# OwshenNetwork/owshen

Hardware: NVIDIA H100
Metric: groth16_withdraw_proofs_per_sec (higher is better)
Workload: dtype u256 (8x32-bit Montgomery limbs, integer)

## Files before the change

### owshen_b200/csrc/ec.cuh

```cuda
#pragma once
#include "fp.cuh"

namespace og {

template <class F>
struct Affine {
    F x, y;
    OG_HD static Affine inf() { return Affine{F::zero(), F::zero()}; }
    OG_HD bool is_inf() const { return x.is_zero() && y.is_zero(); }
    OG_HD Affine neg() const { return Affine{x, y.neg()}; }
    OG_HD bool operator==(const Affine& o) const { return x == o.x && y == o.y; }
};

template <class F>
struct XYZZ {
    F x, y, zz, zzz;

    OG_HD static XYZZ inf() { return XYZZ{F::one(), F::one(), F::zero(), F::zero()}; }
    OG_HD bool is_inf() const { return zz.is_zero(); }
    OG_HD static XYZZ from_affine(const Affine<F>& p) {
        if (p.is_inf()) return inf();
        return XYZZ{p.x, p.y, F::one(), F::one()};
    }
    OG_HD XYZZ neg() const { return XYZZ{x, y.neg(), zz, zzz}; }

    OG_HD static XYZZ dbl_affine(const Affine<F>& p) {
        F u = p.y.dbl();
        F v = u.sqr();
        F w = u * v;
        F s = p.x * v;
        F xx = p.x.sqr();
        F m = xx.dbl() + xx;
        F x3 = m.sqr() - s.dbl();
        F y3 = m * (s - x3) - w * p.y;
        return XYZZ{x3, y3, v, w};
    }

    OG_HD XYZZ dbl() const {
        if (is_inf()) return *this;
        F u = y.dbl();
        F v = u.sqr();
        F w = u * v;
        F s = x * v;
        F xx = x.sqr();
        F m = xx.dbl() + xx;
        F x3 = m.sqr() - s.dbl();
        F y3 = m * (s - x3) - w * y;
        return XYZZ{x3, y3, v * zz, w * zzz};
    }

    OG_HD void madd(const Affine<F>& q) {
        if (q.is_inf()) return;
        if (is_inf()) { x = q.x; y = q.y; zz = F::one(); zzz = F::one(); return; }
        F u2 = q.x * zz;
        F s2 = q.y * zzz;
        F p = u2 - x;
        F r = s2 - y;
        if (p.is_zero()) {
            if (r.is_zero()) *this = dbl_affine(q);
            else *this = inf();
            return;
        }
        F pp = p.sqr();
        F ppp = p * pp;
        F q1 = x * pp;
        F x3 = r.sqr() - ppp - q1.dbl();
        y = r * (q1 - x3) - y * ppp;
        x = x3;
        zz = zz * pp;
        zzz = zzz * ppp;
    }

    OG_HD void add(const XYZZ& o) {
        if (o.is_inf()) return;
        if (is_inf()) { *this = o; return; }
        F u1 = x * o.zz;
        F u2 = o.x * zz;
        F s1 = y * o.zzz;
        F s2 = o.y * zzz;
        F p = u2 - u1;
        F r = s2 - s1;
        if (p.is_zero()) {
            if (r.is_zero()) *this = dbl();
            else *this = inf();
            return;
        }
        F pp = p.sqr();
        F ppp = p * pp;
        F q1 = u1 * pp;
        F x3 = r.sqr() - ppp - q1.dbl();
        y = r * (q1 - x3) - s1 * ppp;
        x = x3;
        zz = zz * o.zz * pp;
        zzz = zzz * o.zzz * ppp;
    }

    OG_HD Affine<F> to_affine() const {
        if (is_inf()) return Affine<F>::inf();
        F t = (zz * zzz).inv();
        return Affine<F>{x * (t * zzz), y * (t * zz)};
    }

    OG_HD static XYZZ mul(const Affine<F>& p, const uint32_t* k) {
        XYZZ acc = inf();
        for (int i = 255; i >= 0; i--) {
            acc = acc.dbl();
            if ((k[i >> 5] >> (i & 31)) & 1) acc.madd(p);
        }
        return acc;
    }
};

#if defined(__CUDACC__)
template <class F> __device__ __noinline__ void xyzz_add_ni(XYZZ<F>* a, const XYZZ<F>* b) { a->add(*b); }
template <class F> __device__ __noinline__ void xyzz_madd_ni(XYZZ<F>* a, const Affine<F>* b) { a->madd(*b); }
template <class F> __device__ __noinline__ void xyzz_dbl_ni(XYZZ<F>* a) { *a = a->dbl(); }
template <class F> __device__ __noinline__ void xyzz_to_affine_ni(Affine<F>* r, const XYZZ<F>* a) { *r = a->to_affine(); }
#endif

typedef Affine<Fq> G1Affine;
typedef Affine<Fq2> G2Affine;
typedef XYZZ<Fq> G1XYZZ;
typedef XYZZ<Fq2> G2XYZZ;

}
```

### owshen_b200/csrc/fp.cuh

```cuda
#pragma once
#include <stdint.h>
#include <string.h>

#if defined(__CUDACC__)
#define OG_HD __host__ __device__ __forceinline__
#else
#define OG_HD inline
#endif

namespace og {

struct CC { uint32_t c = 0; };

#if defined(__CUDA_ARCH__)
#define OG_ASM asm volatile
OG_HD uint32_t add_cc(uint32_t a, uint32_t b, CC&) { uint32_t r; OG_ASM("add.cc.u32 %0, %1, %2;" : "=r"(r) : "r"(a), "r"(b)); return r; }
OG_HD uint32_t addc_cc(uint32_t a, uint32_t b, CC&) { uint32_t r; OG_ASM("addc.cc.u32 %0, %1, %2;" : "=r"(r) : "r"(a), "r"(b)); return r; }
OG_HD uint32_t addc(uint32_t a, uint32_t b, CC&) { uint32_t r; OG_ASM("addc.u32 %0, %1, %2;" : "=r"(r) : "r"(a), "r"(b)); return r; }
OG_HD uint32_t sub_cc(uint32_t a, uint32_t b, CC&) { uint32_t r; OG_ASM("sub.cc.u32 %0, %1, %2;" : "=r"(r) : "r"(a), "r"(b)); return r; }
OG_HD uint32_t subc_cc(uint32_t a, uint32_t b, CC&) { uint32_t r; OG_ASM("subc.cc.u32 %0, %1, %2;" : "=r"(r) : "r"(a), "r"(b)); return r; }
OG_HD uint32_t subc(uint32_t a, uint32_t b, CC&) { uint32_t r; OG_ASM("subc.u32 %0, %1, %2;" : "=r"(r) : "r"(a), "r"(b)); return r; }
OG_HD uint32_t mad_lo_cc(uint32_t a, uint32_t b, uint32_t c, CC&) { uint32_t r; OG_ASM("mad.lo.cc.u32 %0, %1, %2, %3;" : "=r"(r) : "r"(a), "r"(b), "r"(c)); return r; }
OG_HD uint32_t madc_lo_cc(uint32_t a, uint32_t b, uint32_t c, CC&) { uint32_t r; OG_ASM("madc.lo.cc.u32 %0, %1, %2, %3;" : "=r"(r) : "r"(a), "r"(b), "r"(c)); return r; }
OG_HD uint32_t madc_hi_cc(uint32_t a, uint32_t b, uint32_t c, CC&) { uint32_t r; OG_ASM("madc.hi.cc.u32 %0, %1, %2, %3;" : "=r"(r) : "r"(a), "r"(b), "r"(c)); return r; }
// ... 307 lines not shown
    OG_HD static Fp zero() { Fp r; for (int i = 0; i < 8; i++) r.l[i] = 0; return r; }
    OG_HD static Fp one() { Fp r;
#pragma unroll
        for (int i = 0; i < 8; i++) r.l[i] = P::one(i);
        return r; }
    OG_HD bool is_zero() const { uint32_t o = 0;
#pragma unroll
        for (int i = 0; i < 8; i++) o |= l[i];
        return o == 0; }
    OG_HD bool operator==(const Fp& b) const { uint32_t o = 0;
#pragma unroll
        for (int i = 0; i < 8; i++) o |= l[i] ^ b.l[i];
        return o == 0; }
    OG_HD bool operator!=(const Fp& b) const { return !(*this == b); }

    OG_HD friend Fp operator*(const Fp& a, const Fp& b) { Fp r; mont_mul<P>(r.l, a.l, b.l); return r; }
#if defined(OG_SQR_INTERLEAVED)
    OG_HD Fp sqr() const { Fp r; mont_mul<P>(r.l, l, l); return r; }
#else
    OG_HD Fp sqr() const { Fp r; uint32_t T[16]; sqr_wide(T, l); mont_reduce_wide<P>(r.l, T); return r; }
#endif

    OG_HD static Fp mul_lazy(const Fp& a, const Fp& b) { Fp r; mont_mul_lazy<P>(r.l, a.l, b.l); return r; }
    OG_HD Fp sqr_lazy() const { Fp r; uint32_t T[16]; sqr_wide(T, l); mont_reduce_wide_lazy<P>(r.l, T); return r; }
    OG_HD static Fp add_raw(const Fp& a, const Fp& b) {
        Fp r; CC cc;
        r.l[0] = add_cc(a.l[0], b.l[0], cc);
#pragma unroll
        for (int j = 1; j < 7; j++) r.l[j] = addc_cc(a.l[j], b.l[j], cc);
        r.l[7] = addc(a.l[7], b.l[7], cc);
        return r;
    }
    OG_HD Fp reduce_4p_to_2p() const { Fp r = *this; cond_sub_2p<P>(r.l); return r; }
    OG_HD Fp reduce_2p_to_p() const { Fp r = *this; final_sub<P>(r.l); return r; }

    OG_HD friend Fp operator+(const Fp& a, const Fp& b) {
        Fp r; CC cc;
        r.l[0] = add_cc(a.l[0], b.l[0], cc);
#pragma unroll
        for (int j = 1; j < 7; j++) r.l[j] = addc_cc(a.l[j], b.l[j], cc);
        r.l[7] = addc(a.l[7], b.l[7], cc);
        final_sub<P>(r.l);
        return r;
    }
    OG_HD friend Fp operator-(const Fp& a, const Fp& b) {
        Fp r; CC cc;
        r.l[0] = sub_cc(a.l[0], b.l[0], cc);
#pragma unroll
        for (int j = 1; j < 8; j++) r.l[j] = subc_cc(a.l[j], b.l[j], cc);
        uint32_t borrow = subc(0u, 0u, cc);
        r.l[0] = add_cc(r.l[0], P::mod(0) & borrow, cc);
#pragma unroll
        for (int j = 1; j < 7; j++) r.l[j] = addc_cc(r.l[j], P::mod(j) & borrow, cc);
        r.l[7] = addc(r.l[7], P::mod(7) & borrow, cc);
        return r;
    }
    OG_HD Fp neg() const { return zero() - *this; }
    OG_HD Fp dbl() const { return *this + *this; }

    OG_HD static Fp from_canonical(const uint32_t* c) {
        Fp t, r2;
#pragma unroll
        for (int i = 0; i < 8; i++) { t.l[i] = c[i]; r2.l[i] = P::r2(i); }
        return t * r2;
    }
    OG_HD void to_canonical(uint32_t* c) const {
        Fp o = zero(); o.l[0] = 1;
        Fp t = *this * o;
#pragma unroll
        for (int i = 0; i < 8; i++) c[i] = t.l[i];
    }
    OG_HD static bool canonical_lt_mod(const uint32_t* c) {
        for (int i = 7; i >= 0; i--) {
            if (c[i] < P::mod(i)) return true;
            if (c[i] > P::mod(i)) return false;
        }
        return false;
    }
    OG_HD static Fp from_u32(uint32_t v) { uint32_t c[8] = {v, 0, 0, 0, 0, 0, 0, 0}; return from_canonical(c); }

    OG_HD Fp pow(const uint32_t* e) const {
        Fp acc = one();
        for (int i = 255; i >= 0; i--) {
            acc = acc.sqr();
            if ((e[i >> 5] >> (i & 31)) & 1) acc = acc * *this;
        }
        return acc;
    }
    OG_HD Fp inv() const {
        uint32_t e[8];
#pragma unroll
        for (int i = 0; i < 8; i++) e[i] = P::mod(i);
        e[0] -= 2;
        return pow(e);
    }
};

typedef Fp<FqParams> Fq;
typedef Fp<FrParams> Fr;

struct Fq2 {
    Fq c0, c1;
    OG_HD static Fq2 zero() { return Fq2{Fq::zero(), Fq::zero()}; }
    OG_HD static Fq2 one() { return Fq2{Fq::one(), Fq::zero()}; }
    OG_HD bool is_zero() const { return c0.is_zero() && c1.is_zero(); }
    OG_HD bool operator==(const Fq2& b) const { return c0 == b.c0 && c1 == b.c1; }
    OG_HD bool operator!=(const Fq2& b) const { return !(*this == b); }
    OG_HD friend Fq2 operator+(const Fq2& a, const Fq2& b) { return Fq2{a.c0 + b.c0, a.c1 + b.c1}; }
    OG_HD friend Fq2 operator-(const Fq2& a, const Fq2& b) { return Fq2{a.c0 - b.c0, a.c1 - b.c1}; }
    OG_HD static Fq2 mul_inl(const Fq2& a, const Fq2& b) {
        uint32_t T0[16], T1[16], T2[16], sa[8], sb[8];
        CC cc;
        mul_wide(T0, a.c0.l, b.c0.l);
        mul_wide(T1, a.c1.l, b.c1.l);
        sa[0] = add_cc(a.c0.l[0], a.c1.l[0], cc);
        for (int j = 1; j < 7; j++) sa[j] = addc_cc(a.c0.l[j], a.c1.l[j], cc);
        sa[7] = addc(a.c0.l[7], a.c1.l[7], cc);
        sb[0] = add_cc(b.c0.l[0], b.c1.l[0], cc);
        for (int j = 1; j < 7; j++) sb[j] = addc_cc(b.c0.l[j], b.c1.l[j], cc);
        sb[7] = addc(b.c0.l[7], b.c1.l[7], cc);
        mul_wide(T2, sa, sb);
        T2[0] = sub_cc(T2[0], T0[0], cc);
        for (int j = 1; j < 15; j++) T2[j] = subc_cc(T2[j], T0[j], cc);
        T2[15] = subc(T2[15], T0[15], cc);
        T2[0] = sub_cc(T2[0], T1[0], cc);
        for (int j = 1; j < 15; j++) T2[j] = subc_cc(T2[j], T1[j], cc);
        T2[15] = subc(T2[15], T1[15], cc);
        T0[0] = sub_cc(T0[0], T1[0], cc);
        for (int j = 1; j < 15; j++) T0[j] = subc_cc(T0[j], T1[j], cc);
        T0[15] = subc(T0[15], T1[15], cc);
        T0[8] = add_cc(T0[8], FqParams::mod(0), cc);
        for (int j = 1; j < 7; j++) T0[8 + j] = addc_cc(T0[8 + j], FqParams::mod(j), cc);
        T0[15] = addc(T0[15], FqParams::mod(7), cc);
        Fq2 r;
        mont_reduce_wide<FqParams>(r.c0.l, T0);
        final_sub<FqParams>(r.c0.l);
        mont_reduce_wide<FqParams>(r.c1.l, T2);
        return r;
    }
    OG_HD static Fq2 sqr_inl(const Fq2& a) {
        Fq m = a.c0 * a.c1;
        return Fq2{(a.c0 + a.c1) * (a.c0 - a.c1), m + m};
    }
    OG_HD friend Fq2 operator*(const Fq2& a, const Fq2& b);
    OG_HD Fq2 sqr() const;
    OG_HD Fq2 neg() const { return Fq2{c0.neg(), c1.neg()}; }
    OG_HD Fq2 dbl() const { return Fq2{c0.dbl(), c1.dbl()}; }
    OG_HD Fq2 inv() const {
        Fq n = (c0.sqr() + c1.sqr()).inv();
        return Fq2{c0 * n, (c1 * n).neg()};
    }
    OG_HD Fq2 conj() const { return Fq2{c0, c1.neg()}; }
    OG_HD Fq2 mul_fq(const Fq& s) const { return Fq2{c0 * s, c1 * s}; }
};

#if defined(__CUDA_ARCH__) && defined(OG_FP_MUL_CALL)
static __device__ __noinline__ Fq2 fq2_mul_call(Fq2 a, Fq2 b) { return Fq2::mul_inl(a, b); }
static __device__ __noinline__ Fq2 fq2_sqr_call(Fq2 a) { return Fq2::sqr_inl(a); }
OG_HD Fq2 operator*(const Fq2& a, const Fq2& b) { return fq2_mul_call(a, b); }
OG_HD Fq2 Fq2::sqr() const { return fq2_sqr_call(*this); }
#else
OG_HD Fq2 operator*(const Fq2& a, const Fq2& b) { return Fq2::mul_inl(a, b); }
OG_HD Fq2 Fq2::sqr() const { return Fq2::sqr_inl(*this); }
#endif

}
```

### owshen_b200/csrc/msm.cu

```cuda
#include "msm.cuh"
#include "glv.cuh"
#include <stdlib.h>
#if !defined(OG_MSM_G1) && !defined(OG_MSM_G2)
#error "compile msm.cu with -DOG_MSM_G1 or -DOG_MSM_G2"
#endif

namespace og {

template <class F> struct FieldIO;
template <> struct FieldIO<Fq> {
    static constexpr int BYTES = 32;
    static __device__ __forceinline__ Fq load(const uint8_t* p, int* flag) { return load_canonical<Fq>(p, flag); }
    static __device__ __forceinline__ void store(uint8_t* p, const Fq& v) { store_canonical(p, v); }
};
template <> struct FieldIO<Fq2> {
    static constexpr int BYTES = 64;
    static __device__ __forceinline__ Fq2 load(const uint8_t* p, int* flag) {
        return Fq2{load_canonical<Fq>(p, flag), load_canonical<Fq>(p + 32, flag)};
    }
    static __device__ __forceinline__ void store(uint8_t* p, const Fq2& v) { store_canonical(p, v.c0); store_canonical(p + 32, v.c1); }
};

template <class F>
__global__ void __launch_bounds__(128) k_points_to_mont(const uint8_t* __restrict__ in, uint64_t n, Affine<F>* __restrict__ out, int* flag) {
// ... 344 lines not shown
        uint32_t* tile_offs = d_tiles + n_runs;
        uint32_t* stage_e = d_stage;
        uint8_t* stage_f = reinterpret_cast<uint8_t*>(d_stage + (uint64_t)plan.n_problems * plan.n * plan.n_windows);
        dim3 tgrid(n_tiles, plan.n_problems);
        OG_LAUNCH(ctx, k_sort_part_count, tgrid, SORT_THREADS, 0, plan, shift, n_tiles, tile_counts, ctx->d_flag);
        OG_TRY(exclusive_scan(ctx, tile_counts, n_runs, tile_offs, nullptr));
        OG_LAUNCH(ctx, k_sort_part_scatter, tgrid, SORT_THREADS, 0, plan, shift, n_tiles, tile_offs, stage_e, stage_f, ctx->d_flag);
        OG_LAUNCH(ctx, k_sort_local, n_parts, SORT_THREADS, 0, tile_offs, n_tiles, n_parts, shift, tile_offs + n_runs, stage_e, stage_f,
                  d_counts, d_offsets, d_sorted);
        return OG_OK;
    }
    OG_CUDA(ctx, cudaMemsetAsync(d_counts, 0, sizeof(uint32_t) * (size_t)n_keys, ctx->stream));
    dim3 grid((unsigned)((plan.n + 255) / 256), plan.n_problems);
    OG_LAUNCHN(ctx, "k_digits_count", k_digits<false>, grid, 256, 0, plan, d_counts, nullptr, nullptr, nullptr, ctx->d_flag);
    OG_TRY(exclusive_scan(ctx, d_counts, n_keys, d_offsets, d_cursor));
    OG_LAUNCHN(ctx, "k_digits_scatter", k_digits<true>, grid, 256, 0, plan, d_counts, d_offsets, d_cursor, d_sorted, ctx->d_flag);
    return OG_OK;
}
#endif


constexpr uint32_t ORDER_BINS = 2048;
template <class F>
__global__ void __launch_bounds__(1024) k_bucket_order(const uint32_t* __restrict__ counts, uint32_t nb, uint32_t* __restrict__ perm) {
    __shared__ uint32_t hist[ORDER_BINS];
    const uint32_t g = blockIdx.x, t = threadIdx.x;
    const uint32_t* c = counts + (size_t)g * nb;
    for (uint32_t i = t; i < ORDER_BINS; i += 1024) hist[i] = 0;
    __syncthreads();
    for (uint32_t b = t; b < nb; b += 1024) atomicAdd(&hist[ORDER_BINS - 1 - min(c[b], ORDER_BINS - 1)], 1u);
    __syncthreads();
    __shared__ uint32_t pair[1024];
    uint32_t a0 = hist[2 * t], a1 = hist[2 * t + 1];
    pair[t] = a0 + a1;
    __syncthreads();
    for (uint32_t d = 1; d < 1024; d <<= 1) {
        uint32_t v = t >= d ? pair[t - d] : 0;
        __syncthreads();
        pair[t] += v;
        __syncthreads();
    }
    uint32_t base = t ? pair[t - 1] : 0;
    hist[2 * t] = base;
    hist[2 * t + 1] = base + a0;
    __syncthreads();
    for (uint32_t b = t; b < nb; b += 1024) {
        uint32_t pos = atomicAdd(&hist[ORDER_BINS - 1 - min(c[b], ORDER_BINS - 1)], 1u);
        perm[(size_t)g * nb + pos] = g * nb + b;
    }
}

template <class F>
__device__ __forceinline__ Affine<F> fetch_point(const Affine<F>* __restrict__ table, uint32_t e) {
    Affine<F> p = table[e >> 1];
    if (e & 1) p.y = p.y.neg();
    return p;
}

#ifdef OG_MSM_G1
struct SmAcc1 {
    uint4* base;
    __device__ __forceinline__ Fq ld(int coord) const {
        Fq v;
        uint4 a = base[(coord * 2 + 0) * 128], b = base[(coord * 2 + 1) * 128];
        v.l[0] = a.x; v.l[1] = a.y; v.l[2] = a.z; v.l[3] = a.w; v.l[4] = b.x; v.l[5] = b.y; v.l[6] = b.z; v.l[7] = b.w;
        return v;
    }
    __device__ __forceinline__ void st(int coord, const Fq& v) const {
        base[(coord * 2 + 0) * 128] = make_uint4(v.l[0], v.l[1], v.l[2], v.l[3]);
        base[(coord * 2 + 1) * 128] = make_uint4(v.l[4], v.l[5], v.l[6], v.l[7]);
    }
};

#ifndef OG_SQR_CALL
#define OG_SQR_CALL 1
#endif
#if OG_SQR_CALL
static __device__ __noinline__ Fq fq_sqr_call(Fq a) { return a.sqr(); }
#define OG_ACC_SQR(x) fq_sqr_call(x)
#else
#define OG_ACC_SQR(x) (x).sqr()
#endif
#if defined(OG_MUL_CALL) && OG_MUL_CALL
static __device__ __noinline__ Fq fq_mul_call(Fq a, Fq b) { return a * b; }
#define OG_ACC_MUL(x, y) fq_mul_call((x), (y))
#else
#define OG_ACC_MUL(x, y) ((x) * (y))
#endif
#ifndef OG_ACC1_MINB
#define OG_ACC1_MINB 8
#endif
__global__ void __launch_bounds__(128, OG_ACC1_MINB) k_bucket_acc_sm1(const Affine<Fq>* __restrict__ table, const uint32_t* __restrict__ sorted,
                                                        const uint32_t* __restrict__ offsets, const uint32_t* __restrict__ counts,
                                                        uint32_t n_keys, uint32_t cap, XYZZ<Fq>* __restrict__ buckets,
                                                        uint32_t* __restrict__ heavy, const uint32_t* __restrict__ perm) {
    __shared__ uint4 sm_acc[8 * 128];
    uint32_t slot_ = blockIdx.x * blockDim.x + threadIdx.x;
    if (slot_ >= n_keys) return;
    uint32_t key = perm[slot_];
    uint32_t cnt = counts[key], off = offsets[key];
    if (cnt > cap) {
        uint32_t slot = atomicAdd(heavy, 1u);
        heavy[1 + slot] = key;
        buckets[key] = XYZZ<Fq>::inf();
        return;
    }
    SmAcc1 A{sm_acc + threadIdx.x};
    bool inf = true;
    uint32_t e = cnt ? sorted[off] : 0;
    for (uint32_t k = 0; k < cnt; k++) {
        uint32_t en = k + 1 < cnt ? sorted[off + k + 1] : 0;
        Affine<Fq> q = fetch_point(table, e);
        e = en;
        if (q.is_inf()) continue;
        if (inf) { A.st(0, q.x); A.st(1, q.y); A.st(2, Fq::one()); A.st(3, Fq::one()); inf = false; continue; }
        Fq p = OG_ACC_MUL(q.x, A.ld(2)) - A.ld(0);
        Fq r = OG_ACC_MUL(q.y, A.ld(3)) - A.ld(1);
        if (p.is_zero()) {
            if (r.is_zero()) { XYZZ<Fq> d = XYZZ<Fq>::dbl_affine(q); A.st(0, d.x); A.st(1, d.y); A.st(2, d.zz); A.st(3, d.zzz); }
            else inf = true;
            continue;
        }
        Fq pp = OG_ACC_SQR(p);
        A.st(2, OG_ACC_MUL(A.ld(2), pp));
        Fq ppp = OG_ACC_MUL(p, pp);
        A.st(3, OG_ACC_MUL(A.ld(3), ppp));
        Fq q1 = OG_ACC_MUL(A.ld(0), pp);
        Fq x3 = OG_ACC_SQR(r) - ppp - q1.dbl();
        A.st(0, x3);
        A.st(1, OG_ACC_MUL(r, q1 - x3) - OG_ACC_MUL(A.ld(1), ppp));
    }
    buckets[key] = inf ? XYZZ<Fq>::inf() : XYZZ<Fq>{A.ld(0), A.ld(1), A.ld(2), A.ld(3)};
}
#endif

#ifdef OG_MSM_G2
struct SmAcc {
    uint4* base;
    __device__ __forceinline__ Fq2 ld(int coord) const {
        Fq2 v;
        uint4 a = base[(coord * 4 + 0) * 128], b = base[(coord * 4 + 1) * 128], c = base[(coord * 4 + 2) * 128], d = base[(coord * 4 + 3) * 128];
        v.c0.l[0] = a.x; v.c0.l[1] = a.y; v.c0.l[2] = a.z; v.c0.l[3] = a.w; v.c0.l[4] = b.x; v.c0.l[5] = b.y; v.c0.l[6] = b.z; v.c0.l[7] = b.w;
        v.c1.l[0] = c.x; v.c1.l[1] = c.y; v.c1.l[2] = c.z; v.c1.l[3] = c.w; v.c1.l[4] = d.x; v.c1.l[5] = d.y; v.c1.l[6] = d.z; v.c1.l[7] = d.w;
        return v;
    }
    __device__ __forceinline__ void st(int coord, const Fq2& v) const {
        base[(coord * 4 + 0) * 128] = make_uint4(v.c0.l[0], v.c0.l[1], v.c0.l[2], v.c0.l[3]);
        base[(coord * 4 + 1) * 128] = make_uint4(v.c0.l[4], v.c0.l[5], v.c0.l[6], v.c0.l[7]);
        base[(coord * 4 + 2) * 128] = make_uint4(v.c1.l[0], v.c1.l[1], v.c1.l[2], v.c1.l[3]);
        base[(coord * 4 + 3) * 128] = make_uint4(v.c1.l[4], v.c1.l[5], v.c1.l[6], v.c1.l[7]);
    }
};

__global__ void __launch_bounds__(128, 6) k_bucket_acc_sm(const Affine<Fq2>* __restrict__ table, const uint32_t* __restrict__ sorted,
                                                       const uint32_t* __restrict__ offsets, const uint32_t* __restrict__ counts,
                                                       uint32_t n_keys, uint32_t cap, XYZZ<Fq2>* __restrict__ buckets,
                                                       uint32_t* __restrict__ heavy, const uint32_t* __restrict__ perm) {
    __shared__ uint4 sm_acc[16 * 128];
    uint32_t slot_ = blockIdx.x * blockDim.x + threadIdx.x;
    if (slot_ >= n_keys) return;
    uint32_t key = perm[slot_];
    uint32_t cnt = counts[key], off = offsets[key];
    if (cnt > cap) {
        uint32_t slot = atomicAdd(heavy, 1u);
        heavy[1 + slot] = key;
        buckets[key] = XYZZ<Fq2>::inf();
        return;
    }
    SmAcc A{sm_acc + threadIdx.x};
    bool inf = true;
    uint32_t e = cnt ? sorted[off] : 0;
    for (uint32_t k = 0; k < cnt; k++) {
        uint32_t en = k + 1 < cnt ? sorted[off + k + 1] : 0;
        Affine<Fq2> q = fetch_point(table, e);
        e = en;
        if (q.is_inf()) continue;
        if (inf) { A.st(0, q.x); A.st(1, q.y); A.st(2, Fq2::one()); A.st(3, Fq2::one()); inf = false; continue; }
        Fq2 p = q.x * A.ld(2) - A.ld(0);
        Fq2 r = q.y * A.ld(3) - A.ld(1);
        if (p.is_zero()) {
            if (r.is_zero()) { XYZZ<Fq2> d = XYZZ<Fq2>::dbl_affine(q); A.st(0, d.x); A.st(1, d.y); A.st(2, d.zz); A.st(3, d.zzz); }
            else inf = true;
            continue;
        }
        Fq2 pp = p.sqr();
        A.st(2, A.ld(2) * pp);
        Fq2 ppp = p * pp;
        A.st(3, A.ld(3) * ppp);
        Fq2 q1 = A.ld(0) * pp;
        Fq2 x3 = r.sqr() - ppp - q1.dbl();
        A.st(0, x3);
        Fq2 t = A.ld(1) * ppp;
        A.st(1, r * (q1 - x3) - t);
    }
    buckets[key] = inf ? XYZZ<Fq2>::inf() : XYZZ<Fq2>{A.ld(0), A.ld(1), A.ld(2), A.ld(3)};
}
#endif

template <class F>
__global__ void __launch_bounds__(256) k_heavy_plan(uint32_t* __restrict__ heavy, const uint32_t* __restrict__ counts, uint32_t n_keys, uint32_t seg) {
    __shared__ uint32_t part[256];
    __shared__ uint32_t carry;
    const uint32_t n_heavy = heavy[0];
    uint32_t* seg_base = heavy + 1 + n_keys;
    if (threadIdx.x == 0) carry = 0;
    __syncthreads();
    for (uint32_t base = 0; base < n_heavy; base += 256) {
        uint32_t h = base + threadIdx.x;
        uint32_t v = h < n_heavy ? (counts[heavy[1 + h]] + seg - 1) / seg : 0;
        part[threadIdx.x] = v;
        __syncthreads();
        for (uint32_t d = 1; d < 256; d <<= 1) {
            uint32_t t = threadIdx.x >= d ? part[threadIdx.x - d] : 0;
            __syncthreads();
            part[threadIdx.x] += t;
            __syncthreads();
        }
        if (h < n_heavy) seg_base[h] = carry + part[threadIdx.x] - v;
        __syncthreads();
        if (threadIdx.x == 255) carry += part[255];
        __syncthreads();
    }
    if (threadIdx.x == 0) seg_base[n_heavy] = carry;
}

template <class F, int THREADS>
__global__ void __launch_bounds__(THREADS) k_bucket_heavy(const Affine<F>* __restrict__ table, const uint32_t* __restrict__ sorted,
                                                          const uint32_t* __restrict__ offsets, const uint32_t* __restrict__ counts,
                                                          uint32_t n_keys, uint32_t seg, XYZZ<F>* __restrict__ partials,
                                                          const uint32_t* __restrict__ heavy) {
    extern __shared__ __align__(32) unsigned char smem_raw[];
    XYZZ<F>* sh = reinterpret_cast<XYZZ<F>*>(smem_raw);
    const uint32_t n_heavy = heavy[0];
    const uint32_t* seg_base = heavy + 1 + n_keys;
    const uint32_t n_seg = n_heavy ? seg_base[n_heavy] : 0;
    for (uint32_t g = blockIdx.x; g < n_seg; g += gridDim.x) {
        uint32_t lo = 0, hi = n_heavy;
        while (hi - lo > 1) { uint32_t mid = (lo + hi) >> 1; if (seg_base[mid] <= g) lo = mid; else hi = mid; }
        const uint32_t key = heavy[1 + lo];
        const uint32_t cnt = counts[key], off = offsets[key];
        const uint32_t k0 = (g - seg_base[lo]) * seg, k1 = k0 + seg < cnt ? k0 + seg : cnt;
        XYZZ<F> acc = XYZZ<F>::inf();
        for (uint32_t k = k0 + threadIdx.x; k < k1; k += THREADS) { Affine<F> q = fetch_point(table, sorted[off + k]); xyzz_madd_ni(&acc, &q); }
        sh[threadIdx.x] = acc;
        __syncthreads();
        for (int s = THREADS / 2; s > 0; s >>= 1) {
            if ((int)threadIdx.x < s) xyzz_add_ni(&sh[threadIdx.x], &sh[threadIdx.x + s]);
            __syncthreads();
        }
        if (threadIdx.x == 0) partials[g] = sh[0];
        __syncthreads();
    }
}

template <class F>
__global__ void __launch_bounds__(32) k_heavy_combine(const XYZZ<F>* __restrict__ partials, uint32_t n_keys, XYZZ<F>* __restrict__ buckets,
                                                      const uint32_t* __restrict__ heavy) {
    __shared__ XYZZ<F> sh[32];
    const uint32_t n_heavy = heavy[0];
    const uint32_t* seg_base = heavy + 1 + n_keys;
    for (uint32_t h = blockIdx.x; h < n_heavy; h += gridDim.x) {
        const uint32_t s0 = seg_base[h], s1 = seg_base[h + 1];
        XYZZ<F> acc = XYZZ<F>::inf();
        for (uint32_t s = s0 + threadIdx.x; s < s1; s += 32) xyzz_add_ni(&acc, &partials[s]);
        sh[threadIdx.x] = acc;
        __syncwarp();
        for (int w = 16; w > 0; w >>= 1) {
            if ((int)threadIdx.x < w) xyzz_add_ni(&sh[threadIdx.x], &sh[threadIdx.x + w]);
            __syncwarp();
        }
        if (threadIdx.x == 0) buckets[heavy[1 + h]] = sh[0];
        __syncwarp();
    }
}

#ifdef OG_EXPERIMENT_AFFINE
#include "experiments/bucket_affine.cuh"
#endif

constexpr uint32_t RED_FAN_LOG2 = 3, RED_FAN = 1u << RED_FAN_LOG2;
template <class F> struct RedOps {
    static __device__ __forceinline__ void add(XYZZ<F>& a, const XYZZ<F>& b) { a.add(b); }
    static __device__ __forceinline__ void dbl(XYZZ<F>& a) { a = a.dbl(); }
};
#ifdef OG_MSM_G1
static __device__ __noinline__ XYZZ<Fq> g1_add_rv(XYZZ<Fq> a, XYZZ<Fq> b) { a.add(b); return a; }
static __device__ __noinline__ XYZZ<Fq> g1_dbl_rv(XYZZ<Fq> a) { return a.dbl(); }
template <> struct RedOps<Fq> {
    static __device__ __forceinline__ void add(XYZZ<Fq>& a, const XYZZ<Fq>& b) { a = g1_add_rv(a, b); }
    static __device__ __forceinline__ void dbl(XYZZ<Fq>& a) { a = g1_dbl_rv(a); }
};
#endif

template <class F> constexpr bool RED_SM_DEFAULT = sizeof(F) != 32;

template <class F, bool HAS_U>
__global__ void __launch_bounds__(64) k_reduce_level(const XYZZ<F>* __restrict__ S_in, const XYZZ<F>* __restrict__ U_in,
                                                     uint32_t n_in, uint32_t n_out, uint32_t n_groups, uint32_t w_log2,
                                                     uint32_t fan_log2, XYZZ<F>* __restrict__ S_out, XYZZ<F>* __restrict__ U_out) {
    uint32_t t = blockIdx.x * blockDim.x + threadIdx.x;
    if (t >= n_groups * n_out) return;
    uint32_t g = t / n_out, p = t % n_out;
    const XYZZ<F>* S = S_in + (size_t)g * n_in;
    uint32_t lo = p << fan_log2, hi = min(n_in, lo + (1u << fan_log2));
    XYZZ<F> R = XYZZ<F>::inf(), T = XYZZ<F>::inf();
    for (uint32_t i = hi - 1; i > lo; i--) {
        RedOps<F>::add(R, S[i]);
        RedOps<F>::add(T, R);
    }
    RedOps<F>::add(R, S[lo]);
    for (uint32_t k = 0; k < w_log2; k++) RedOps<F>::dbl(T);
    if (HAS_U) {
        const XYZZ<F>* U = U_in + (size_t)g * n_in;
        for (uint32_t i = lo; i < hi; i++) RedOps<F>::add(T, U[i]);
    }
    S_out[(size_t)g * n_out + p] = R;
    U_out[(size_t)g * n_out + p] = T;
}

template <class F> struct RedSm {
    static constexpr int CH = sizeof(F) / 16, THREADS = 64;
    uint4* base;
    __device__ __forceinline__ F ld(int acc, int coord) const {
        F v; uint32_t* w = reinterpret_cast<uint32_t*>(&v);
#pragma unroll
        for (int c = 0; c < CH; c++) { uint4 q = base[((acc * 4 + coord) * CH + c) * THREADS]; w[4 * c] = q.x; w[4 * c + 1] = q.y; w[4 * c + 2] = q.z; w[4 * c + 3] = q.w; }
        return v;
    }
    __device__ __forceinline__ void st(int acc, int coord, const F& v) const {
        const uint32_t* w = reinterpret_cast<const uint32_t*>(&v);
#pragma unroll
        for (int c = 0; c < CH; c++) base[((acc * 4 + coord) * CH + c) * THREADS] = make_uint4(w[4 * c], w[4 * c + 1], w[4 * c + 2], w[4 * c + 3]);
    }
};
template <class F> struct RedGlobalOp {
    const XYZZ<F>* p;
    __device__ __forceinline__ bool inf() const { return p->zz.is_zero(); }
    __device__ __forceinline__ F coord(int c) const { return c == 0 ? p->x : (c == 1 ? p->y : (c == 2 ? p->zz : p->zzz)); }
};
template <class F> struct RedSmOp {
    RedSm<F> M; int acc; bool is_inf;
    __device__ __forceinline__ bool inf() const { return is_inf; }
    __device__ __forceinline__ F coord(int c) const { return M.ld(acc, c); }
};

template <class F, class Op>
__device__ __forceinline__ void red_sm_add(const RedSm<F>& M, int a, bool& a_inf, const Op& o) {
    if (o.inf()) return;
// ... 538 lines not shown
```

Measured before the change: 1648.

## Use lazy-reduced Fq2 arithmetic in G2 bucket accumulation and relax launch bounds

Adds lazy-reduction Fq2 helpers that keep values in [0, 2p), defer final subtraction, and fold the Karatsuba subtraction into a single wide reduction. The G2 shared-memory bucket accumulation kernel now uses these through a new g2_madd_lazy routine and canonicalises the results only at the end. This is meant to cut conditional subtractions and reductions per mixed addition. It also lowers the kernel's minimum blocks per SM from 6 to 4, which frees registers but may reduce occupancy. The lazy zero checks must recognise both 0 and p as zero to stay correct.

```diff
diff --git a/owshen_b200/csrc/ec.cuh b/owshen_b200/csrc/ec.cuh
--- a/owshen_b200/csrc/ec.cuh
+++ b/owshen_b200/csrc/ec.cuh
@@ -111,6 +111,28 @@
     }
 };
 
+template <class Acc>
+OG_HD bool g2_madd_lazy(const Acc& A, const Affine<Fq2>& q) {
+    Fq2 p = Fq2::sub_lazy(fq2_mul_lazy(q.x, A.ld(2)), A.ld(0));
+    Fq2 r = Fq2::sub_lazy(fq2_mul_lazy(q.y, A.ld(3)), A.ld(1));
+    if (p.is_zero_lazy()) {
+        if (!r.is_zero_lazy()) return false;
+        XYZZ<Fq2> d = XYZZ<Fq2>::dbl_affine(q);
+        A.st(0, d.x); A.st(1, d.y); A.st(2, d.zz); A.st(3, d.zzz);
+        return true;
+    }
+    Fq2 pp = fq2_sqr_lazy(p);
+    A.st(2, fq2_mul_lazy(A.ld(2), pp));
+    Fq2 ppp = fq2_mul_lazy(p, pp);
+    A.st(3, fq2_mul_lazy(A.ld(3), ppp));
+    Fq2 q1 = fq2_mul_lazy(A.ld(0), pp);
+    Fq2 x3 = Fq2::sub_lazy(Fq2::sub_lazy(fq2_sqr_lazy(r), ppp), Fq2::add_lazy(q1, q1));
+    A.st(0, x3);
+    Fq2 t = fq2_mul_lazy(A.ld(1), ppp);
+    A.st(1, Fq2::sub_lazy(fq2_mul_lazy(r, Fq2::sub_lazy(q1, x3)), t));
+    return true;
+}
+
 #if defined(__CUDACC__)
 template <class F> __device__ __noinline__ void xyzz_add_ni(XYZZ<F>* a, const XYZZ<F>* b) { a->add(*b); }
 template <class F> __device__ __noinline__ void xyzz_madd_ni(XYZZ<F>* a, const Affine<F>* b) { a->madd(*b); }
diff --git a/owshen_b200/csrc/fp.cuh b/owshen_b200/csrc/fp.cuh
--- a/owshen_b200/csrc/fp.cuh
+++ b/owshen_b200/csrc/fp.cuh
@@ -483,6 +483,99 @@
     }
     OG_HD Fq2 conj() const { return Fq2{c0, c1.neg()}; }
     OG_HD Fq2 mul_fq(const Fq& s) const { return Fq2{c0 * s, c1 * s}; }
+
+    OG_HD static void add_lazy_fq(uint32_t* r, const uint32_t* a, const uint32_t* b) {
+        CC cc;
+        r[0] = add_cc(a[0], b[0], cc);
+#pragma unroll
+        for (int j = 1; j < 7; j++) r[j] = addc_cc(a[j], b[j], cc);
+        r[7] = addc(a[7], b[7], cc);
+        cond_sub_2p<FqParams>(r);
+    }
+    OG_HD static void sub_lazy_fq(uint32_t* r, const uint32_t* a, const uint32_t* b) {
+        CC cc;
+        r[0] = sub_cc(a[0], b[0], cc);
+#pragma unroll
+        for (int j = 1; j < 8; j++) r[j] = subc_cc(a[j], b[j], cc);
+        uint32_t borrow = subc(0u, 0u, cc);
+        r[0] = add_cc(r[0], mod2<FqParams>(0) & borrow, cc);
+#pragma unroll
+        for (int j = 1; j < 7; j++) r[j] = addc_cc(r[j], mod2<FqParams>(j) & borrow, cc);
+        r[7] = addc(r[7], mod2<FqParams>(7) & borrow, cc);
+    }
+    OG_HD static void sub_raw_fq(uint32_t* r, const uint32_t* a, const uint32_t* b) {
+        CC cc;
+        r[0] = add_cc(a[0], mod2<FqParams>(0), cc);
+#pragma unroll
+        for (int j = 1; j < 7; j++) r[j] = addc_cc(a[j], mod2<FqParams>(j), cc);
+        r[7] = addc(a[7], mod2<FqParams>(7), cc);
+        r[0] = sub_cc(r[0], b[0], cc);
+#pragma unroll
+        for (int j = 1; j < 7; j++) r[j] = subc_cc(r[j], b[j], cc);
+        r[7] = subc(r[7], b[7], cc);
+    }
+    OG_HD static bool is_zero_lazy_fq(const uint32_t* a) {
+        uint32_t z = 0, q = 0;
+#pragma unroll
+        for (int j = 0; j < 8; j++) { z |= a[j]; q |= a[j] ^ FqParams::mod(j); }
+        return z == 0 || q == 0;
+    }
+    OG_HD static Fq2 add_lazy(const Fq2& a, const Fq2& b) { Fq2 r; add_lazy_fq(r.c0.l, a.c0.l, b.c0.l); add_lazy_fq(r.c1.l, a.c1.l, b.c1.l); return r; }
+    OG_HD static Fq2 sub_lazy(const Fq2& a, const Fq2& b) { Fq2 r; sub_lazy_fq(r.c0.l, a.c0.l, b.c0.l); sub_lazy_fq(r.c1.l, a.c1.l, b.c1.l); return r; }
+    OG_HD bool is_zero_lazy() const { return is_zero_lazy_fq(c0.l) && is_zero_lazy_fq(c1.l); }
+    OG_HD Fq2 canonical() const { Fq2 r = *this; final_sub<FqParams>(r.c0.l); final_sub<FqParams>(r.c1.l); return r; }
+
+    OG_HD static Fq2 mul_lazy_inl(const Fq2& a, const Fq2& b) {
+        uint32_t T0[16], T1[16], S[16];
+        CC cc;
+        mul_wide(T0, a.c0.l, b.c0.l);
+        mul_wide(T1, a.c1.l, b.c1.l);
+        S[0] = add_cc(T0[0], T1[0], cc);
+#pragma unroll
+        for (int j = 1; j < 15; j++) S[j] = addc_cc(T0[j], T1[j], cc);
+        S[15] = addc(T0[15], T1[15], cc);
+        T0[0] = sub_cc(T0[0], T1[0], cc);
+#pragma unroll
+        for (int j = 1; j < 15; j++) T0[j] = subc_cc(T0[j], T1[j], cc);
+        T0[15] = subc(T0[15], T1[15], cc);
+        T0[8] = add_cc(T0[8], FqParams::mod(0), cc);
+#pragma unroll
+        for (int j = 1; j < 7; j++) T0[8 + j] = addc_cc(T0[8 + j], FqParams::mod(j), cc);
+        T0[15] = addc(T0[15], FqParams::mod(7), cc);
+        Fq2 r;
+        mont_reduce_wide_lazy<FqParams>(r.c0.l, T0);
+        cond_sub_2p<FqParams>(r.c0.l);
+        uint32_t sa[8], sb[8];
+        sa[0] = add_cc(a.c0.l[0], a.c1.l[0], cc);
+#pragma unroll
+        for (int j = 1; j < 7; j++) sa[j] = addc_cc(a.c0.l[j], a.c1.l[j], cc);
+        sa[7] = addc(a.c0.l[7], a.c1.l[7], cc);
+        sb[0] = add_cc(b.c0.l[0], b.c1.l[0], cc);
+#pragma unroll
+        for (int j = 1; j < 7; j++) sb[j] = addc_cc(b.c0.l[j], b.c1.l[j], cc);
+        sb[7] = addc(b.c0.l[7], b.c1.l[7], cc);
+        mul_wide(T1, sa, sb);
+        T1[0] = sub_cc(T1[0], S[0], cc);
+#pragma unroll
+        for (int j = 1; j < 15; j++) T1[j] = subc_cc(T1[j], S[j], cc);
+        T1[15] = subc(T1[15], S[15], cc);
+        mont_reduce_wide_lazy<FqParams>(r.c1.l, T1);
+        cond_sub_2p<FqParams>(r.c1.l);
+        return r;
+    }
+    OG_HD static Fq2 sqr_lazy_inl(const Fq2& a) {
+        uint32_t T[16], u[8], v[8];
+        Fq2 r;
+        mul_wide(T, a.c0.l, a.c1.l);
+        mont_reduce_wide_lazy<FqParams>(r.c1.l, T);
+        add_lazy_fq(r.c1.l, r.c1.l, r.c1.l);
+        add_lazy_fq(u, a.c0.l, a.c1.l);
+        sub_raw_fq(v, a.c0.l, a.c1.l);
+        mul_wide(T, u, v);
+        mont_reduce_wide_lazy<FqParams>(r.c0.l, T);
+        cond_sub_2p<FqParams>(r.c0.l);
+        return r;
+    }
 };
 
 #if defined(__CUDA_ARCH__) && defined(OG_FP_MUL_CALL)
@@ -495,4 +588,14 @@
 OG_HD Fq2 Fq2::sqr() const { return Fq2::sqr_inl(*this); }
 #endif
 
-}
+#if defined(__CUDA_ARCH__) && defined(OG_FP_MUL_CALL)
+static __device__ __noinline__ Fq2 fq2_mul_lazy_call(Fq2 a, Fq2 b) { return Fq2::mul_lazy_inl(a, b); }
+static __device__ __noinline__ Fq2 fq2_sqr_lazy_call(Fq2 a) { return Fq2::sqr_lazy_inl(a); }
+OG_HD Fq2 fq2_mul_lazy(const Fq2& a, const Fq2& b) { return fq2_mul_lazy_call(a, b); }
+OG_HD Fq2 fq2_sqr_lazy(const Fq2& a) { return fq2_sqr_lazy_call(a); }
+#else
+OG_HD Fq2 fq2_mul_lazy(const Fq2& a, const Fq2& b) { return Fq2::mul_lazy_inl(a, b); }
+OG_HD Fq2 fq2_sqr_lazy(const Fq2& a) { return Fq2::sqr_lazy_inl(a); }
+#endif
+
+}
diff --git a/owshen_b200/csrc/msm.cu b/owshen_b200/csrc/msm.cu
--- a/owshen_b200/csrc/msm.cu
+++ b/owshen_b200/csrc/msm.cu
@@ -520,7 +520,10 @@
     }
 };
 
-__global__ void __launch_bounds__(128, 6) k_bucket_acc_sm(const Affine<Fq2>* __restrict__ table, const uint32_t* __restrict__ sorted,
+#ifndef OG_ACC2_MINB
+#define OG_ACC2_MINB 4
+#endif
+__global__ void __launch_bounds__(128, OG_ACC2_MINB) k_bucket_acc_sm(const Affine<Fq2>* __restrict__ table, const uint32_t* __restrict__ sorted,
                                                        const uint32_t* __restrict__ offsets, const uint32_t* __restrict__ counts,
                                                        uint32_t n_keys, uint32_t cap, XYZZ<Fq2>* __restrict__ buckets,
                                                        uint32_t* __restrict__ heavy, const uint32_t* __restrict__ perm) {
@@ -544,24 +547,9 @@
         e = en;
         if (q.is_inf()) continue;
         if (inf) { A.st(0, q.x); A.st(1, q.y); A.st(2, Fq2::one()); A.st(3, Fq2::one()); inf = false; continue; }
-        Fq2 p = q.x * A.ld(2) - A.ld(0);
-        Fq2 r = q.y * A.ld(3) - A.ld(1);
-        if (p.is_zero()) {
-            if (r.is_zero()) { XYZZ<Fq2> d = XYZZ<Fq2>::dbl_affine(q); A.st(0, d.x); A.st(1, d.y); A.st(2, d.zz); A.st(3, d.zzz); }
-            else inf = true;
-            continue;
-        }
-        Fq2 pp = p.sqr();
-        A.st(2, A.ld(2) * pp);
-        Fq2 ppp = p * pp;
-        A.st(3, A.ld(3) * ppp);
-        Fq2 q1 = A.ld(0) * pp;
-        Fq2 x3 = r.sqr() - ppp - q1.dbl();
-        A.st(0, x3);
-        Fq2 t = A.ld(1) * ppp;
-        A.st(1, r * (q1 - x3) - t);
-    }
-    buckets[key] = inf ? XYZZ<Fq2>::inf() : XYZZ<Fq2>{A.ld(0), A.ld(1), A.ld(2), A.ld(3)};
+        if (!g2_madd_lazy(A, q)) inf = true;
+    }
+    buckets[key] = inf ? XYZZ<Fq2>::inf() : XYZZ<Fq2>{A.ld(0).canonical(), A.ld(1).canonical(), A.ld(2).canonical(), A.ld(3).canonical()};
 }
 #endif
 
```

After: 1774 (median of 6 runs). 1.08x the previous value.
